# comprna/RATTLE

Hardware: AMD Instinct MI355X
Metric: reads/sec for `cluster`+`correct` on 1e6×1kb synthetic ONT reads, 1→8 GPU (higher is better)
Workload: dtype int16

## Files before the change

rattle_amd/csrc/post_msa.hip:

```cpp
#include <cmath>
#include <cstring>

#include "common.h"

namespace rattle {

__device__ __forceinline__ uint8_t d_comp_base(uint8_t c) {
    switch (c) {
        case 'A': return 'T';
        case 'C': return 'G';
        case 'T': return 'A';
        case 'G': return 'C';
        case 'U': return 'A';
    }
    return c;
}

__global__ __launch_bounds__(256) void gather_kernel(const gather_desc *D, uint32_t n, const uint8_t *sseq, const uint8_t *squal,
                                                      uint8_t *dseq, uint8_t *dqual) {
    const uint32_t w = blockIdx.x * 4u + (threadIdx.x >> 6), lane = threadIdx.x & 63u;
    if (w >= n) return;
    const gather_desc d = D[w];
    if (d.flags & 1u) {
        for (uint32_t t = lane; t < d.len; t += 64) {
            const uint64_t s = d.src + d.len - 1 - t;
            dseq[d.dst + t] = d_comp_base(sseq[s]);
            if (dqual) dqual[d.dst + t] = squal[s];
        }
    } else {
        for (uint32_t t = lane; t < d.len; t += 64) {
            dseq[d.dst + t] = sseq[d.src + t];
            if (dqual) dqual[d.dst + t] = squal[d.src + t];
        }
    }
}

int launch_gather(rattle_ctx *ctx, const gather_desc *d_desc, uint32_t n, const uint8_t *sseq, const uint8_t *squal, uint8_t *dseq,
                  uint8_t *dqual) {
    if (n == 0) return 0;
    hipLaunchKernelGGL(gather_kernel, dim3((n + 3) / 4), dim3(256), 0, ctx->stream, d_desc, n, sseq, squal, dseq, dqual);
    RT_HIP(hipGetLastError());
    return 0;
}

__device__ int phred_value(const post_args &A, double p) {
    const unsigned long long bits = (unsigned long long)__double_as_longlong(p);
    int a = 0, b = (int)A.n_exc;
    while (a < b) { const int m = (a + b) >> 1; if (A.exc_bits[m] < bits) a = m + 1; else b = m; }
    if (a < (int)A.n_exc && A.exc_bits[a] == bits) return A.exc_val[a];
    int lo = 0, hi = A.phred_cnt - 1;
    while (lo < hi) { const int m = (lo + hi) >> 1; if (p >= A.phred_lo[m]) hi = m; else lo = m + 1; }
    return A.phred_n0 + lo;
}

template <bool REV>
__device__ void fix_phase(uint8_t *r, uint32_t n, uint32_t &trimmed, uint32_t &stop_pos, bool &stopped) {
#define AT(p) (REV ? r[n - 1u - (p)] : r[(p)])
    uint32_t pos = 0;
    trimmed = 0; stopped = false; stop_pos = n;
    while (pos < n) {
        while (pos < n && AT(pos) == '-') ++pos;
        uint32_t end = pos;
        int gaps = 0, sz = 0;
        while (gaps < 4 && end < n) {
            if (AT(end) == '-') ++gaps; else { ++sz; gaps = 0; }
            ++end;
        }
        if (sz < 10) {
            while (end < n && AT(end) == '-') { ++end; ++gaps; }
            if (gaps >= 20) {
                for (uint32_t t = pos; t < end; ++t) { if (REV) r[n - 1u - t] = '-'; else r[t] = '-'; }
                trimmed += (uint32_t)sz;
                pos = end;
                continue;
            }
        }
        stopped = true; stop_pos = pos;
        break;
    }
#undef AT
}

__device__ __forceinline__ void vote_support(const post_args &A, uint32_t p, uint32_t tid, uint32_t q0, uint32_t R, uint32_t W, const uint8_t *rc,
                                             const uint32_t *msup, const uint32_t *mdep) {
    uint8_t *ccons = A.ccons + A.coff[p];
    uint32_t *ccnt = A.ccnt + A.coff[p];
    uint8_t o[6];
    for (int s = 0; s < 6; ++s) o[s] = A.order[s];
    for (uint32_t k = tid; k < W; k += 256) {
        uint32_t occ[6] = {0, 0, 0, 0, 0, 0}, sup[6] = {0, 0, 0, 0, 0, 0}, dep = 0;
        for (uint32_t i = 0; i < R; ++i) {
            if ((int32_t)k < A.rfirst[q0 + i] || (int32_t)k > A.rlast[q0 + i]) continue;
            const uint8_t nt = rc[(uint64_t)i * W + k];
            const uint32_t sv = !msup ? 1u : nt != '-' ? msup[(uint64_t)i * W + k] : 0u;
            dep += msup ? mdep[(uint64_t)i * W + k] : 1u;
#pragma unroll
            for (int s = 0; s < 6; ++s) if (nt == o[s]) { ++occ[s]; sup[s] += sv; }
        }
        uint32_t best = 0, bsup = 0, total = 0;
        uint8_t nt = 0;
#pragma unroll
        for (int s = 0; s < 6; ++s) { total += occ[s]; if (occ[s] > best) { best = occ[s]; nt = o[s]; bsup = sup[s]; } }
        ccons[k] = nt ? nt : (uint8_t)'-';
        ccnt[k] = bsup; ccnt[A.cnt_stride + k] = dep; ccnt[2 * A.cnt_stride + k] = best; ccnt[3 * A.cnt_stride + k] = total;
    }
}

template <int MODE, bool REPORT = false>
__global__ __launch_bounds__(256) void post_msa_kernel(post_args A) {
    constexpr bool SUPPORT = MODE == 2 && REPORT;
    __shared__ double s_perr[256];
    const uint32_t p = blockIdx.x, tid = threadIdx.x;
    const uint32_t q0 = A.pack_first[p], q1 = A.pack_first[p + 1], R = q1 - q0;
    const uint32_t W = A.width[p];
    uint8_t *rc = A.rowc + A.moff[p];
    uint8_t *rq = MODE == 1 ? A.rowq + A.moff[p] : nullptr;
    const uint64_t cells = (uint64_t)R * W;
    if (MODE == 1) s_perr[tid] = A.perr[tid];
    if (R == 0 || W == 0) {
        if (tid == 0 && MODE == 2) A.cons_len[p] = 0;
        if (MODE == 1) for (uint32_t i = tid; i < R; i += 256) { A.olen[q0 + i] = 0; A.tfront[q0 + i] = 0; A.tback[q0 + i] = 0; }
        if (REPORT && MODE == 1) for (uint32_t i = tid; i < R; i += 256) for (uint32_t f = 0; f < REP_KERNEL; ++f) A.rep[(uint64_t)f * A.rep_stride + q0 + i] = 0;
        return;
    }
    for (uint64_t t = tid; t < cells; t += 256) { rc[t] = '-'; if (MODE == 1) rq[t] = 0; }
    __syncthreads();
    for (uint32_t i = tid >> 6; i < R; i += 4) {
        const uint64_t b0 = A.off[q0 + i], b1 = A.off[q0 + i + 1];
        uint8_t *row = rc + (uint64_t)i * W;
        for (uint64_t b = b0 + (tid & 63u); b < b1; b += 64) {
            const uint32_t c = A.col[b];
            row[c] = A.seq[b];
            if (MODE == 1) rq[(uint64_t)i * W + c] = A.qual[b];
            if constexpr (SUPPORT) if (p < A.n_composed) { A.msup[A.moff[p] + (uint64_t)i * W + c] = A.in_sup[b]; A.mdep[A.moff[p] + (uint64_t)i * W + c] = A.in_dep[b]; }
        }
    }
    __syncthreads();
    for (uint32_t i = tid; i < R; i += 256) {
        uint8_t *row = rc + (uint64_t)i * W;
        uint32_t t1 = 0, t2 = 0, p1 = W, p2 = W;
        bool s1 = false, s2 = false;
        fix_phase<false>(row, W, t1, p1, s1);
        if (s1) fix_phase<true>(row, W, t2, p2, s2);
        int32_t first = (int32_t)W, last = -1;
        if (s1 && s2 && p1 < W && p2 < W) { first = (int32_t)p1; last = (int32_t)(W - 1u - p2); }
        A.rfirst[q0 + i] = first; A.rlast[q0 + i] = last;
        if (MODE == 1) { A.tfront[q0 + i] = t1; A.tback[q0 + i] = t2; }
        if constexpr (SUPPORT) if (p < A.n_composed) {
            uint32_t *drow = A.mdep + A.moff[p] + (uint64_t)i * W;
            uint32_t carry = 0;
            for (int32_t k = first; k <= last; ++k) { if (row[k] != '-') carry = drow[k]; else drow[k] = carry; }
        }
    }
    __syncthreads();
    uint8_t *ccons = A.ccons + A.coff[p];
    uint8_t *cflag = A.cflag + A.coff[p];
    uint8_t *csym = A.csym + A.coff[p];
    double *cerr = A.cerr + A.coff[p];
    const uint8_t o0 = A.order[0], o1 = A.order[1], o2 = A.order[2], o3 = A.order[3], o4 = A.order[4], o5 = A.order[5];
    if constexpr (SUPPORT) vote_support(A, p, tid, q0, R, W, rc, p < A.n_composed ? A.msup + A.moff[p] : nullptr, p < A.n_composed ? A.mdep + A.moff[p] : nullptr);
    else for (uint32_t k = tid; k < W; k += 256) {
        int occ0 = 0, occ1 = 0, occ2 = 0, occ3 = 0, occ4 = 0, occ5 = 0;
        double e0 = 0.0, e1 = 0.0, e2 = 0.0, e3 = 0.0, e4 = 0.0, e5 = 0.0;
        for (uint32_t i = 0; i < R; ++i) {
            if ((int32_t)k < A.rfirst[q0 + i] || (int32_t)k > A.rlast[q0 + i]) continue;
            const uint8_t nt = rc[(uint64_t)i * W + k];
            if (MODE == 1) {
                const double ep = nt != '-' ? s_perr[rq[(uint64_t)i * W + k]] : 0.0;
                if (nt == o0) { ++occ0; e0 += ep; } else if (nt == o1) { ++occ1; e1 += ep; } else if (nt == o2) { ++occ2; e2 += ep; }
                else if (nt == o3) { ++occ3; e3 += ep; } else if (nt == o4) { ++occ4; e4 += ep; } else if (nt == o5) { ++occ5; e5 += ep; }
            } else {
                occ0 += nt == o0; occ1 += nt == o1; occ2 += nt == o2; occ3 += nt == o3; occ4 += nt == o4; occ5 += nt == o5;
            }
        }
        const int total = occ0 + occ1 + occ2 + occ3 + occ4 + occ5;
        int best = 0, bocc = 0;
        uint8_t nt = 0;
        double berr = 0.0;
#define SLOT(occ, err, oc)                                                      \
        { double m = err; if (occ > 0 && MODE == 1) m = err / double(occ);      \
          if (occ > best) { best = occ; nt = oc; bocc = occ; berr = m; } }
        SLOT(occ0, e0, o0) SLOT(occ1, e1, o1) SLOT(occ2, e2, o2) SLOT(occ3, e3, o3) SLOT(occ4, e4, o4) SLOT(occ5, e5, o5)
#undef SLOT
        if (nt == 0) { ccons[k] = '-'; if (MODE == 1) { cflag[k] = 0; csym[k] = 0; cerr[k] = 0.0; } continue; }
        ccons[k] = nt;
        if (MODE == 1) {
            const double ratio = double(bocc) / double(total);
            cflag[k] = (uint8_t)((ratio >= A.gap_occ ? 1 : 0) | (ratio >= A.min_occ ? 2 : 0));
            cerr[k] = berr;
            csym[k] = (uint8_t)(phred_value(A, berr) & 0xFF);
        }
    }
    __syncthreads();
    if (MODE == 1) {
        for (uint32_t i = tid; i < R; i += 256) {
            uint8_t *row = rc + (uint64_t)i * W;
            uint8_t *qrow = rq + (uint64_t)i * W;
            const int32_t first = A.rfirst[q0 + i], last = A.rlast[q0 + i];
            uint32_t o = 0;
            uint32_t n_match = 0, n_subst = 0, n_miskept = 0, n_ins = 0, n_del = 0, n_gapkept = 0;
            for (int32_t k = first; k <= last; ++k) {
                const uint8_t nt = row[k], qq = qrow[k], cnt = ccons[k], fl = cflag[k];
                uint8_t es = 0, eq = 0;
                bool emit = true;
                if (cnt == '-') {
                    if (nt != '-' && !(fl & 1)) { es = nt; eq = qq; if (REPORT) ++n_gapkept; }
                    else { emit = false; if (REPORT && nt != '-') ++n_del; }
                } else if (nt == '-') {
                    if (fl & 1) { es = cnt; eq = csym[k]; if (REPORT) ++n_ins; } else emit = false;
                } else if (nt == cnt) {
                    es = nt; eq = qq;
                    if (REPORT) ++n_match;
                } else if ((fl & 2) && A.err_ratio * s_perr[qq] > cerr[k]) {
                    es = cnt; eq = csym[k];
                    if (REPORT) ++n_subst;
                } else {
                    es = nt; eq = qq;
                    if (REPORT) ++n_miskept;
                }
                if (emit) { row[o] = es; qrow[o] = eq; ++o; }
            }
            A.olen[q0 + i] = o;
            if (REPORT) {
                uint32_t *rep = A.rep + q0 + i;
                const uint64_t s = A.rep_stride;
                rep[(REP_MATCH - REP_MATCH) * s] = n_match; rep[(REP_SUBST - REP_MATCH) * s] = n_subst; rep[(REP_MISKEPT - REP_MATCH) * s] = n_miskept;
                rep[(REP_INS - REP_MATCH) * s] = n_ins; rep[(REP_DEL - REP_MATCH) * s] = n_del; rep[(REP_GAPKEPT - REP_MATCH) * s] = n_gapkept;
            }
        }
    } else {
        if (tid < 64) {
            uint8_t *out = A.cons_out + A.coff[p];
            uint32_t o = 0;
            for (uint32_t base = 0; base < W; base += 64) {
                const uint32_t k = base + tid;
                const uint8_t c = k < W ? ccons[k] : (uint8_t)'-';
                const bool keep = c != '-';
                const unsigned long long m = __ballot(keep);
                if (keep) out[o + __popcll(m & ((1ull << tid) - 1ull))] = c;
                if constexpr (SUPPORT) if (keep) {
                    const uint32_t *cc = A.ccnt + A.coff[p] + k;
                    uint32_t *oc = A.ocnt + A.coff[p] + o + __popcll(m & ((1ull << tid) - 1ull));
                    for (uint32_t f = 0; f < 4; ++f) oc[f * A.cnt_stride] = cc[f * A.cnt_stride];
                }
                o += (uint32_t)__popcll(m);
            }
            if (tid == 0) A.cons_len[p] = o;
        }
    }
}

int launch_post_msa(rattle_ctx *ctx, const post_args &A, uint32_t n_packs, int mode) {
    if (n_packs == 0) return 0;
    ktimer T(ctx, K_POST, 0);
    if (mode == 1 && A.rep) hipLaunchKernelGGL((post_msa_kernel<1, true>), dim3(n_packs), dim3(256), 0, ctx->stream, A);
    else if (mode == 1) hipLaunchKernelGGL(post_msa_kernel<1>, dim3(n_packs), dim3(256), 0, ctx->stream, A);
    else if (A.ccnt) hipLaunchKernelGGL((post_msa_kernel<2, true>), dim3(n_packs), dim3(256), 0, ctx->stream, A);
    else hipLaunchKernelGGL(post_msa_kernel<2>, dim3(n_packs), dim3(256), 0, ctx->stream, A);
    RT_HIP(hipGetLastError());
    return 0;
}

namespace {
inline int phred_host(double p) { return (int)(-10 * log10(p) + 33); }
inline double from_bits(uint64_t b) { double d; memcpy(&d, &b, 8); return d; }
}

void build_phred_table(phred_table &T) {
    T.n0 = -300;
    const int cnt = 700;
    T.lo.assign(cnt, 0.0);
    T.exc_bits.clear(); T.exc_val.clear();
    const uint64_t bmin = 1, bmax = 0x7FEFFFFFFFFFFFFFull;
    for (int t = 0; t < cnt; ++t) {
        const int n = T.n0 + t;
        uint64_t a = bmin, b = bmax;
        while (a < b) { const uint64_t m = a + (b - a) / 2; if (phred_host(from_bits(m)) <= n) b = m; else a = m + 1; }
        T.lo[t] = from_bits(a);
    }
    auto table_value = [&](double p) {
        int lo = 0, hi = cnt - 1;
        while (lo < hi) { const int m = (lo + hi) >> 1; if (p >= T.lo[m]) hi = m; else lo = m + 1; }
        return T.n0 + lo;
    };
    std::vector<std::pair<uint64_t, int>> exc;
    for (int t = 0; t < cnt; ++t) {
        uint64_t c; memcpy(&c, &T.lo[t], 8);
        if (c < 4096 || c > bmax - 4096) continue;
        for (uint64_t b = c - 2048; b <= c + 2048; ++b) {
            const double p = from_bits(b);
            const int want = phred_host(p);
            if (table_value(p) != want) exc.emplace_back(b, want);
        }
    }
    std::sort(exc.begin(), exc.end());
    exc.erase(std::unique(exc.begin(), exc.end()), exc.end());
    for (auto &e : exc) { T.exc_bits.push_back(e.first); T.exc_val.push_back(e.second); }
}

int phred_lookup_host(const phred_table &T, double p) {
    uint64_t bits;
    memcpy(&bits, &p, 8);
    const auto it = std::lower_bound(T.exc_bits.begin(), T.exc_bits.end(), bits);
    if (it != T.exc_bits.end() && *it == bits) return T.exc_val[it - T.exc_bits.begin()];
    int lo = 0, hi = (int)T.lo.size() - 1;
    while (lo < hi) { const int m = (lo + hi) >> 1; if (p >= T.lo[m]) hi = m; else lo = m + 1; }
    return T.n0 + lo;
}

}
```

Before: 218,500.

## Restructure post-MSA kernel around wave-cooperative rows and LDS-staged scatter

```diff
diff --git a/rattle_amd/csrc/post_msa.hip b/rattle_amd/csrc/post_msa.hip
--- a/rattle_amd/csrc/post_msa.hip
+++ b/rattle_amd/csrc/post_msa.hip
@@ -53,32 +53,66 @@
     return A.phred_n0 + lo;
 }
 
+constexpr uint32_t POST_WAVES = 4;
+constexpr uint32_t POST_WIN_ROWS = 1024;
+constexpr uint32_t POST_STAGE_W = 2048;
+constexpr int POST_VOTE_COLS = 4;
+constexpr int POST_FIX_BLOCKS = 4;
+
+__device__ __forceinline__ uint32_t wave_uniform(uint32_t v) { return (uint32_t)__builtin_amdgcn_readfirstlane((int)v); }
+
+__device__ __forceinline__ uint32_t wave_sum(uint32_t v) {
+#pragma unroll
+    for (int s = 32; s > 0; s >>= 1) v += (uint32_t)__shfl_xor((int)v, s);
+    return v;
+}
+
 template <bool REV>
-__device__ void fix_phase(uint8_t *r, uint32_t n, uint32_t &trimmed, uint32_t &stop_pos, bool &stopped) {
-#define AT(p) (REV ? r[n - 1u - (p)] : r[(p)])
-    uint32_t pos = 0;
+__device__ void fix_wave(uint8_t *r, uint32_t n, uint32_t lane, uint32_t start, uint32_t floor, uint32_t &trimmed, uint32_t &stop_pos,
+                         bool &stopped) {
+    uint32_t wbase = 0;
+    unsigned long long m = 0;
+    bool loaded = false;
+    auto base_at = [&](uint32_t p) -> bool {
+        if (!loaded || p - wbase >= 64u) {
+            wbase = p & ~63u; loaded = true;
+            const uint32_t q = wbase + lane;
+            bool b = false;
+            if (q < n) { const uint32_t c = REV ? n - 1u - q : q; b = c >= floor && r[c] != '-'; }
+            m = __ballot(b);
+        }
+        return (m >> (p - wbase)) & 1ull;
+    };
+    auto skip_gaps = [&](uint32_t pos) -> uint32_t {
+        while (pos < n && !base_at(pos)) {
+            const unsigned long long rest = m >> (pos - wbase);
+            pos = rest ? pos + (uint32_t)__builtin_ctzll(rest) : wbase + 64u;
+        }
+        return pos < n ? pos : n;
+    };
     trimmed = 0; stopped = false; stop_pos = n;
+    uint32_t pos = skip_gaps(start < n ? start : n);
+    if (pos >= n) { stopped = true; return; }
     while (pos < n) {
-        while (pos < n && AT(pos) == '-') ++pos;
         uint32_t end = pos;
         int gaps = 0, sz = 0;
-        while (gaps < 4 && end < n) {
-            if (AT(end) == '-') ++gaps; else { ++sz; gaps = 0; }
+        while (gaps < 4 && end < n && sz < 10) {
+            if (!base_at(end)) ++gaps; else { ++sz; gaps = 0; }
             ++end;
         }
         if (sz < 10) {
-            while (end < n && AT(end) == '-') { ++end; ++gaps; }
+            uint32_t run = end;
+            while (run < n && gaps < 20 && !base_at(run)) { ++run; ++gaps; }
             if (gaps >= 20) {
-                for (uint32_t t = pos; t < end; ++t) { if (REV) r[n - 1u - t] = '-'; else r[t] = '-'; }
+                for (uint32_t t = pos + lane; t < end; t += 64) r[REV ? n - 1u - t : t] = '-';
                 trimmed += (uint32_t)sz;
-                pos = end;
+                pos = skip_gaps(run);
                 continue;
             }
         }
         stopped = true; stop_pos = pos;
         break;
     }
-#undef AT
 }
 
 __device__ __forceinline__ void vote_support(const post_args &A, uint32_t p, uint32_t tid, uint32_t q0, uint32_t R, uint32_t W, const uint8_t *rc,
@@ -106,11 +140,50 @@
     }
 }
 
+__device__ __forceinline__ void wave_sync() {
+    __builtin_amdgcn_fence(__ATOMIC_RELEASE, "wavefront");
+    __builtin_amdgcn_wave_barrier();
+    __builtin_amdgcn_fence(__ATOMIC_ACQUIRE, "wavefront");
+}
+
+#ifdef POST_MSA_TICKS
+__device__ unsigned long long g_post_ticks[4];
+#define POST_TICK_BEGIN unsigned long long t_prev = wall_clock64();
+#define POST_TICK(n) do { if (tid == 0) { const unsigned long long t_now = wall_clock64(); atomicAdd(&g_post_ticks[n], t_now - t_prev); t_prev = t_now; } } while (0)
+#else
+#define POST_TICK_BEGIN
+#define POST_TICK(n) do {} while (0)
+#endif
+
+template <int MODE>
+__device__ __forceinline__ void scatter_row(const post_args &A, uint64_t b0, uint64_t b1, uint32_t lane, uint32_t W, uint8_t *dc, uint8_t *dq,
+                                            uint32_t *dsup, uint32_t *ddep) {
+    for (uint64_t b = b0 + lane; b < b1; b += 256) {
+        uint32_t c[4];
+        uint8_t sv[4], qv[4];
+#pragma unroll
+        for (int u = 0; u < 4; ++u) {
+            const uint64_t bu = b + 64u * u < b1 ? b + 64u * u : b;
+            c[u] = A.col[bu]; sv[u] = A.seq[bu]; qv[u] = MODE == 1 ? A.qual[bu] : 0;
+        }
+#pragma unroll
+        for (int u = 0; u < 4; ++u) {
+            if (b + 64u * u >= b1 || c[u] >= W) continue;
+            dc[c[u]] = sv[u];
+            if (MODE == 1) dq[c[u]] = qv[u];
+            if (dsup) { dsup[c[u]] = A.in_sup[b + 64u * u]; ddep[c[u]] = A.in_dep[b + 64u * u]; }
+        }
+    }
+}
+
 template <int MODE, bool REPORT = false>
 __global__ __launch_bounds__(256) void post_msa_kernel(post_args A) {
     constexpr bool SUPPORT = MODE == 2 && REPORT;
     __shared__ double s_perr[256];
-    const uint32_t p = blockIdx.x, tid = threadIdx.x;
+    __shared__ int32_t s_first[POST_WIN_ROWS], s_last[POST_WIN_ROWS];
+    __shared__ uint4 s_rowc[POST_WAVES][POST_STAGE_W / 16 + 2];
+    __shared__ uint4 s_rowq[MODE == 1 ? POST_WAVES : 1][MODE == 1 ? POST_STAGE_W / 16 + 2 : 1];
+    const uint32_t p = blockIdx.x, tid = threadIdx.x, lane = tid & 63u, wave = wave_uniform(tid >> 6);
     const uint32_t q0 = A.pack_first[p], q1 = A.pack_first[p + 1], R = q1 - q0;
     const uint32_t W = A.width[p];
     uint8_t *rc = A.rowc + A.moff[p];
@@ -123,109 +196,199 @@
         if (REPORT && MODE == 1) for (uint32_t i = tid; i < R; i += 256) for (uint32_t f = 0; f < REP_KERNEL; ++f) A.rep[(uint64_t)f * A.rep_stride + q0 + i] = 0;
         return;
     }
-    for (uint64_t t = tid; t < cells; t += 256) { rc[t] = '-'; if (MODE == 1) rq[t] = 0; }
+    POST_TICK_BEGIN
+    const uint4 gap16 = make_uint4(0x2d2d2d2du, 0x2d2d2d2du, 0x2d2d2d2du, 0x2d2d2d2du), zero16 = make_uint4(0u, 0u, 0u, 0u);
+    const bool composed = SUPPORT && p < A.n_composed;
+    if (W <= POST_STAGE_W) {
+        uint4 *l16c = s_rowc[wave], *l16q = s_rowq[MODE == 1 ? wave : 0];
+        uint8_t *lc = reinterpret_cast<uint8_t *>(l16c), *lq = reinterpret_cast<uint8_t *>(l16q);
+        for (uint32_t i = wave; i < R; i += POST_WAVES) {
+            const uint64_t at = (uint64_t)i * W;
+            const uint32_t s = (uint32_t)(at & 15u), nline = (s + W + 15u) >> 4;
+            for (uint32_t j = lane; j < nline; j += 64) { l16c[j] = gap16; if (MODE == 1) l16q[j] = zero16; }
+            wave_sync();
+            const uint64_t b0 = A.off[q0 + i], b1 = A.off[q0 + i + 1];
+            scatter_row<MODE>(A, b0, b1, lane, W, lc + s, MODE == 1 ? lq + s : nullptr, composed ? A.msup + A.moff[p] + at : nullptr, composed ? A.mdep + A.moff[p] + at : nullptr);
+            wave_sync();
+            uint8_t *gc = rc + at - s, *gq = MODE == 1 ? rq + at - s : nullptr;
+            for (uint32_t j = lane; j < nline; j += 64) {
+                const uint32_t x0 = 16u * j;
+                if (x0 >= s && x0 + 16u <= s + W) {
+                    *reinterpret_cast<uint4 *>(gc + x0) = l16c[j];
+                    if (MODE == 1) *reinterpret_cast<uint4 *>(gq + x0) = l16q[j];
+                } else {
+                    for (uint32_t x = x0 < s ? s : x0; x < x0 + 16u && x < s + W; ++x) { gc[x] = lc[x]; if (MODE == 1) gq[x] = lq[x]; }
+                }
+            }
+            wave_sync();
+        }
+    } else {
+        uint4 *c16 = reinterpret_cast<uint4 *>(rc), *q16 = reinterpret_cast<uint4 *>(rq);
+        const uint64_t nline = (cells + 15u) >> 4;
+        for (uint64_t t = tid; t < nline; t += 256) { c16[t] = gap16; if (MODE == 1) q16[t] = zero16; }
+        __syncthreads();
+        for (uint32_t i = wave; i < R; i += POST_WAVES) {
+            const uint64_t at = (uint64_t)i * W;
+            const uint64_t b0 = A.off[q0 + i], b1 = A.off[q0 + i + 1];
+            scatter_row<MODE>(A, b0, b1, lane, W, rc + at, MODE == 1 ? rq + at : nullptr, composed ? A.msup + A.moff[p] + at : nullptr, composed ? A.mdep + A.moff[p] + at : nullptr);
+        }
+    }
     __syncthreads();
-    for (uint32_t i = tid >> 6; i < R; i += 4) {
+    POST_TICK(0);
+    for (uint32_t i = wave; i < R; i += POST_WAVES) {
+        uint8_t *row = rc + (uint64_t)i * W;
         const uint64_t b0 = A.off[q0 + i], b1 = A.off[q0 + i + 1];
-        uint8_t *row = rc + (uint64_t)i * W;
-        for (uint64_t b = b0 + (tid & 63u); b < b1; b += 64) {
-            const uint32_t c = A.col[b];
-            row[c] = A.seq[b];
-            if (MODE == 1) rq[(uint64_t)i * W + c] = A.qual[b];
-            if constexpr (SUPPORT) if (p < A.n_composed) { A.msup[A.moff[p] + (uint64_t)i * W + c] = A.in_sup[b]; A.mdep[A.moff[p] + (uint64_t)i * W + c] = A.in_dep[b]; }
-        }
-    }
-    __syncthreads();
-    for (uint32_t i = tid; i < R; i += 256) {
-        uint8_t *row = rc + (uint64_t)i * W;
+        uint32_t c_first = W, c_last = 0;
+        if (b1 > b0) { c_first = wave_uniform(A.col[b0]); c_last = wave_uniform(A.col[b1 - 1]); }
         uint32_t t1 = 0, t2 = 0, p1 = W, p2 = W;
         bool s1 = false, s2 = false;
-        fix_phase<false>(row, W, t1, p1, s1);
-        if (s1) fix_phase<true>(row, W, t2, p2, s2);
+        fix_wave<false>(row, W, lane, c_first, 0u, t1, p1, s1);
+        if (s1) fix_wave<true>(row, W, lane, b1 > b0 && c_last < W ? W - 1u - c_last : 0u, p1, t2, p2, s2);
         int32_t first = (int32_t)W, last = -1;
         if (s1 && s2 && p1 < W && p2 < W) { first = (int32_t)p1; last = (int32_t)(W - 1u - p2); }
-        A.rfirst[q0 + i] = first; A.rlast[q0 + i] = last;
-        if (MODE == 1) { A.tfront[q0 + i] = t1; A.tback[q0 + i] = t2; }
-        if constexpr (SUPPORT) if (p < A.n_composed) {
+        if (lane == 0) {
+            A.rfirst[q0 + i] = first; A.rlast[q0 + i] = last;
+            if (i < POST_WIN_ROWS) { s_first[i] = first; s_last[i] = last; }
+            if (MODE == 1) { A.tfront[q0 + i] = t1; A.tback[q0 + i] = t2; }
+        }
+        if constexpr (SUPPORT) if (composed) {
             uint32_t *drow = A.mdep + A.moff[p] + (uint64_t)i * W;
             uint32_t carry = 0;
-            for (int32_t k = first; k <= last; ++k) { if (row[k] != '-') carry = drow[k]; else drow[k] = carry; }
+            for (int32_t kb = first; kb <= last; kb += 64) {
+                const int32_t k = kb + (int32_t)lane;
+                const bool in = k <= last, base = in && row[k] != '-';
+                const uint32_t v = base ? drow[k] : 0u;
+                const unsigned long long mb = __ballot(base), below = mb & (~0ull >> (63u - lane));
+                const uint32_t from_block = (uint32_t)__shfl((int)v, below ? 63 - __builtin_clzll(below) : 0);
+                if (in && !base) drow[k] = below ? from_block : carry;
+                const uint32_t top = (uint32_t)__shfl((int)v, mb ? 63 - __builtin_clzll(mb) : 0);
+                if (mb) carry = top;
+            }
         }
     }
     __syncthreads();
+    POST_TICK(1);
     uint8_t *ccons = A.ccons + A.coff[p];
     uint8_t *cflag = A.cflag + A.coff[p];
     uint8_t *csym = A.csym + A.coff[p];
     double *cerr = A.cerr + A.coff[p];
     const uint8_t o0 = A.order[0], o1 = A.order[1], o2 = A.order[2], o3 = A.order[3], o4 = A.order[4], o5 = A.order[5];
     if constexpr (SUPPORT) vote_support(A, p, tid, q0, R, W, rc, p < A.n_composed ? A.msup + A.moff[p] : nullptr, p < A.n_composed ? A.mdep + A.moff[p] : nullptr);
-    else for (uint32_t k = tid; k < W; k += 256) {
-        int occ0 = 0, occ1 = 0, occ2 = 0, occ3 = 0, occ4 = 0, occ5 = 0;
-        double e0 = 0.0, e1 = 0.0, e2 = 0.0, e3 = 0.0, e4 = 0.0, e5 = 0.0;
-        for (uint32_t i = 0; i < R; ++i) {
-            if ((int32_t)k < A.rfirst[q0 + i] || (int32_t)k > A.rlast[q0 + i]) continue;
-            const uint8_t nt = rc[(uint64_t)i * W + k];
-            if (MODE == 1) {
-                const double ep = nt != '-' ? s_perr[rq[(uint64_t)i * W + k]] : 0.0;
-                if (nt == o0) { ++occ0; e0 += ep; } else if (nt == o1) { ++occ1; e1 += ep; } else if (nt == o2) { ++occ2; e2 += ep; }
-                else if (nt == o3) { ++occ3; e3 += ep; } else if (nt == o4) { ++occ4; e4 += ep; } else if (nt == o5) { ++occ5; e5 += ep; }
-            } else {
-                occ0 += nt == o0; occ1 += nt == o1; occ2 += nt == o2; occ3 += nt == o3; occ4 += nt == o4; occ5 += nt == o5;
-            }
-        }
-        const int total = occ0 + occ1 + occ2 + occ3 + occ4 + occ5;
-        int best = 0, bocc = 0;
-        uint8_t nt = 0;
-        double berr = 0.0;
-#define SLOT(occ, err, oc)                                                      \
-        { double m = err; if (occ > 0 && MODE == 1) m = err / double(occ);      \
-          if (occ > best) { best = occ; nt = oc; bocc = occ; berr = m; } }
-        SLOT(occ0, e0, o0) SLOT(occ1, e1, o1) SLOT(occ2, e2, o2) SLOT(occ3, e3, o3) SLOT(occ4, e4, o4) SLOT(occ5, e5, o5)
+    else for (uint32_t k0 = tid * POST_VOTE_COLS; k0 < W; k0 += 256 * POST_VOTE_COLS) {
+        static_assert(POST_VOTE_COLS == 4, "one dword of cells per row");
+#define VOTE_SUMS(c) int occ0_##c = 0, occ1_##c = 0, occ2_##c = 0, occ3_##c = 0, occ4_##c = 0, occ5_##c = 0; \
+                     double e0_##c = 0.0, e1_##c = 0.0, e2_##c = 0.0, e3_##c = 0.0, e4_##c = 0.0, e5_##c = 0.0;
+        VOTE_SUMS(0) VOTE_SUMS(1) VOTE_SUMS(2) VOTE_SUMS(3)
+#undef VOTE_SUMS
+        const uint8_t *pc = rc + k0, *pq = MODE == 1 ? rq + k0 : nullptr;
+#define VOTE_CELL(c)                                                                                                                        \
+            if ((int32_t)k0 + c >= first && (int32_t)k0 + c <= last) {                                                                      \
+                const uint8_t nt = (uint8_t)(vc >> (8 * c));                                                                                \
+                if (MODE == 1) {                                                                                                            \
+                    const double ep = nt != '-' ? s_perr[(vq >> (8 * c)) & 0xFFu] : 0.0;                                                    \
+                                                           \
+                    if (nt == o0) { ++occ0_##c; e0_##c += ep; } else if (nt == o1) { ++occ1_##c; e1_##c += ep; }                            \
+                    else if (nt == o2) { ++occ2_##c; e2_##c += ep; } else if (nt == o3) { ++occ3_##c; e3_##c += ep; }                       \
+                    else if (nt == o4) { ++occ4_##c; e4_##c += ep; } else if (nt == o5) { ++occ5_##c; e5_##c += ep; }                       \
+                } else {                                                                                                                    \
+                    occ0_##c += nt == o0; occ1_##c += nt == o1; occ2_##c += nt == o2; occ3_##c += nt == o3; occ4_##c += nt == o4; occ5_##c += nt == o5; \
+                }                                                                                                                           \
+            }
+#define VOTE_ROW(i, first_of_row, last_of_row)                                  \
+        {                                                                       \
+            const int32_t first = first_of_row, last = last_of_row;             \
+            uint32_t vc, vq = 0;                                                \
+            __builtin_memcpy(&vc, pc + (uint64_t)(i) * W, 4);                   \
+            if (MODE == 1) __builtin_memcpy(&vq, pq + (uint64_t)(i) * W, 4);    \
+            VOTE_CELL(0) VOTE_CELL(1) VOTE_CELL(2) VOTE_CELL(3)                 \
+        }
+        const uint32_t R_lds = R < POST_WIN_ROWS ? R : POST_WIN_ROWS;
+#pragma unroll 4
+        for (uint32_t i = 0; i < R_lds; ++i) VOTE_ROW(i, s_first[i], s_last[i])
+#pragma unroll 1
+        for (uint32_t i = R_lds; i < R; ++i) VOTE_ROW(i, A.rfirst[q0 + i], A.rlast[q0 + i])
+#undef VOTE_ROW
+#undef VOTE_CELL
+#define SLOT(occ, err, oc)                                                          \
+            { double m = err; if (occ > 0 && MODE == 1) m = err / double(occ);      \
+              if (occ > best) { best = occ; nt = oc; bocc = occ; berr = m; } }
+#define VOTE_COLUMN(c)                                                                                                                      \
+        if (k0 + c < W) {                                                                                                                   \
+            const uint32_t k = k0 + c;                                                                                                      \
+            const int total = occ0_##c + occ1_##c + occ2_##c + occ3_##c + occ4_##c + occ5_##c;                                              \
+            int best = 0, bocc = 0;                                                                                                         \
+            uint8_t nt = 0;                                                                                                                 \
+            double berr = 0.0;                                                                                                              \
+            SLOT(occ0_##c, e0_##c, o0) SLOT(occ1_##c, e1_##c, o1) SLOT(occ2_##c, e2_##c, o2)                                                \
+            SLOT(occ3_##c, e3_##c, o3) SLOT(occ4_##c, e4_##c, o4) SLOT(occ5_##c, e5_##c, o5)                                                \
+            if (nt == 0) { ccons[k] = '-'; if (MODE == 1) { cflag[k] = 0; csym[k] = 0; cerr[k] = 0.0; } }                                   \
+            else {                                                                                                                          \
+                ccons[k] = nt;                                                                                                              \
+                if (MODE == 1) {                                                                                                            \
+                    const double ratio = double(bocc) / double(total);                                                                      \
+                    cflag[k] = (uint8_t)((ratio >= A.gap_occ ? 1 : 0) | (ratio >= A.min_occ ? 2 : 0));                                      \
+                    cerr[k] = berr;                                                                                                         \
+                    csym[k] = (uint8_t)(phred_value(A, berr) & 0xFF);                                                                       \
+                }                                                                                                                           \
+            }                                                                                                                               \
+        }
+        VOTE_COLUMN(0) VOTE_COLUMN(1) VOTE_COLUMN(2) VOTE_COLUMN(3)
+#undef VOTE_COLUMN
 #undef SLOT
-        if (nt == 0) { ccons[k] = '-'; if (MODE == 1) { cflag[k] = 0; csym[k] = 0; cerr[k] = 0.0; } continue; }
-        ccons[k] = nt;
-        if (MODE == 1) {
-            const double ratio = double(bocc) / double(total);
-            cflag[k] = (uint8_t)((ratio >= A.gap_occ ? 1 : 0) | (ratio >= A.min_occ ? 2 : 0));
-            cerr[k] = berr;
-            csym[k] = (uint8_t)(phred_value(A, berr) & 0xFF);
-        }
     }
     __syncthreads();
+    POST_TICK(2);
     if (MODE == 1) {
-        for (uint32_t i = tid; i < R; i += 256) {
+        for (uint32_t i = wave; i < R; i += POST_WAVES) {
             uint8_t *row = rc + (uint64_t)i * W;
             uint8_t *qrow = rq + (uint64_t)i * W;
-            const int32_t first = A.rfirst[q0 + i], last = A.rlast[q0 + i];
+            const int32_t first = (int32_t)wave_uniform((uint32_t)A.rfirst[q0 + i]), last = (int32_t)wave_uniform((uint32_t)A.rlast[q0 + i]);
             uint32_t o = 0;
             uint32_t n_match = 0, n_subst = 0, n_miskept = 0, n_ins = 0, n_del = 0, n_gapkept = 0;
-            for (int32_t k = first; k <= last; ++k) {
-                const uint8_t nt = row[k], qq = qrow[k], cnt = ccons[k], fl = cflag[k];
-                uint8_t es = 0, eq = 0;
-                bool emit = true;
-                if (cnt == '-') {
-                    if (nt != '-' && !(fl & 1)) { es = nt; eq = qq; if (REPORT) ++n_gapkept; }
-                    else { emit = false; if (REPORT && nt != '-') ++n_del; }
-                } else if (nt == '-') {
-                    if (fl & 1) { es = cnt; eq = csym[k]; if (REPORT) ++n_ins; } else emit = false;
-                } else if (nt == cnt) {
-                    es = nt; eq = qq;
-                    if (REPORT) ++n_match;
-                } else if ((fl & 2) && A.err_ratio * s_perr[qq] > cerr[k]) {
-                    es = cnt; eq = csym[k];
-                    if (REPORT) ++n_subst;
-                } else {
-                    es = nt; eq = qq;
-                    if (REPORT) ++n_miskept;
+            for (int32_t kb = first; kb <= last; kb += 64 * POST_FIX_BLOCKS) {
+                uint8_t nt[POST_FIX_BLOCKS], qq[POST_FIX_BLOCKS], cnt[POST_FIX_BLOCKS], fl[POST_FIX_BLOCKS], sy[POST_FIX_BLOCKS];
+                double ce[POST_FIX_BLOCKS];
+#pragma unroll
+                for (int u = 0; u < POST_FIX_BLOCKS; ++u) {
+                    const int32_t k = kb + 64 * u + (int32_t)lane, kk = k <= last ? k : last;
+                    nt[u] = row[kk]; qq[u] = qrow[kk]; cnt[u] = ccons[kk]; fl[u] = cflag[kk]; sy[u] = csym[kk]; ce[u] = cerr[kk];
                 }
-                if (emit) { row[o] = es; qrow[o] = eq; ++o; }
-            }
-            A.olen[q0 + i] = o;
+#pragma unroll
+                for (int u = 0; u < POST_FIX_BLOCKS; ++u) {
+                    const int32_t k = kb + 64 * u + (int32_t)lane;
+                    uint8_t es = 0, eq = 0;
+                    bool emit = k <= last;
+                    if (!emit) {
+                    } else if (cnt[u] == '-') {
+                        if (nt[u] != '-' && !(fl[u] & 1)) { es = nt[u]; eq = qq[u]; if (REPORT) ++n_gapkept; }
+                        else { emit = false; if (REPORT && nt[u] != '-') ++n_del; }
+                    } else if (nt[u] == '-') {
+                        if (fl[u] & 1) { es = cnt[u]; eq = sy[u]; if (REPORT) ++n_ins; } else emit = false;
+                    } else if (nt[u] == cnt[u]) {
+                        es = nt[u]; eq = qq[u];
+                        if (REPORT) ++n_match;
+                    } else if ((fl[u] & 2) && A.err_ratio * s_perr[qq[u]] > ce[u]) {
+                        es = cnt[u]; eq = sy[u];
+                        if (REPORT) ++n_subst;
+                    } else {
+                        es = nt[u]; eq = qq[u];
+                        if (REPORT) ++n_miskept;
+                    }
+                    const unsigned long long m = __ballot(emit);
+                    if (emit) { const uint32_t at = o + (uint32_t)__popcll(m & ((1ull << lane) - 1ull)); row[at] = es; qrow[at] = eq; }
+                    o += (uint32_t)__popcll(m);
+                }
+            }
+            if (lane == 0) A.olen[q0 + i] = o;
             if (REPORT) {
-                uint32_t *rep = A.rep + q0 + i;
-                const uint64_t s = A.rep_stride;
-                rep[(REP_MATCH - REP_MATCH) * s] = n_match; rep[(REP_SUBST - REP_MATCH) * s] = n_subst; rep[(REP_MISKEPT - REP_MATCH) * s] = n_miskept;
-                rep[(REP_INS - REP_MATCH) * s] = n_ins; rep[(REP_DEL - REP_MATCH) * s] = n_del; rep[(REP_GAPKEPT - REP_MATCH) * s] = n_gapkept;
+                n_match = wave_sum(n_match); n_subst = wave_sum(n_subst); n_miskept = wave_sum(n_miskept);
+                n_ins = wave_sum(n_ins); n_del = wave_sum(n_del); n_gapkept = wave_sum(n_gapkept);
+                if (lane == 0) {
+                    uint32_t *rep = A.rep + q0 + i;
+                    const uint64_t s = A.rep_stride;
+                    rep[(REP_MATCH - REP_MATCH) * s] = n_match; rep[(REP_SUBST - REP_MATCH) * s] = n_subst; rep[(REP_MISKEPT - REP_MATCH) * s] = n_miskept;
+                    rep[(REP_INS - REP_MATCH) * s] = n_ins; rep[(REP_DEL - REP_MATCH) * s] = n_del; rep[(REP_GAPKEPT - REP_MATCH) * s] = n_gapkept;
+                }
             }
         }
     } else {
@@ -248,10 +411,24 @@
             if (tid == 0) A.cons_len[p] = o;
         }
     }
+    POST_TICK(3);
 }
 
 int launch_post_msa(rattle_ctx *ctx, const post_args &A, uint32_t n_packs, int mode) {
     if (n_packs == 0) return 0;
+    if (((uintptr_t)A.rowc | (uintptr_t)A.rowq) & 15u) { set_error("post-MSA kernel: the row matrices are not 16-byte aligned"); return RATTLE_ERR_HIP; }
+#ifdef POST_MSA_TICKS
+    unsigned long long ticks[4] = {0, 0, 0, 0};
+    RT_HIP(hipMemcpyToSymbol(HIP_SYMBOL(g_post_ticks), ticks, sizeof(ticks)));
+    struct report {
+        rattle_ctx *ctx; int mode; uint32_t n_packs;
+        ~report() {
+            unsigned long long t[4] = {0, 0, 0, 0};
+            if (hipStreamSynchronize(ctx->stream) != hipSuccess || hipMemcpyFromSymbol(t, HIP_SYMBOL(g_post_ticks), sizeof(t)) != hipSuccess) return;
+            fprintf(stderr, "post_msa ticks (10 ns, summed over workgroups): mode %d packs %u a %llu b %llu c %llu d %llu\n", mode, n_packs, t[0], t[1], t[2], t[3]);
+        }
+    } rep{ctx, mode, n_packs};
+#endif
     ktimer T(ctx, K_POST, 0);
     if (mode == 1 && A.rep) hipLaunchKernelGGL((post_msa_kernel<1, true>), dim3(n_packs), dim3(256), 0, ctx->stream, A);
     else if (mode == 1) hipLaunchKernelGGL(post_msa_kernel<1>, dim3(n_packs), dim3(256), 0, ctx->stream, A);
```

Result: faster. 222,200, median of 6 (+1.7%).
